# hyperconnect/TC-ResNet

Measured on AMD Instinct MI355X. Metric: utterances/sec (1 s@16 kHz) TCResNet8-1.0 forward, higher is better.
Workload: dtype f32; 1 GPU; TCResNet8-1.0 eval forward, waveform->softmax, batch 4096/GPU, 49x40 MFCC (40/20 ms, FFT 1024), 12 classes; global_batch=4096, parallelism=dp1 (utterance shards, no collective)

## Files before the change

### tc-resnet_amd/csrc/frontend_pk3.hip

```cpp
#include "frontend_plan.h"
#include "frontend_args.h"

namespace tcr {


namespace {

template <class T> __device__ __forceinline__ T lds_read_unpaired(const T* p) {
    const T v = *p;
    asm volatile("" ::: "memory");
    return v;
}

__device__ __forceinline__ void pk3_dft4(v2& a, v2& b, v2& c, v2& d) {
    const v2 t0 = a + c, t1 = a - c, t2 = b + d, t3 = b - d;
    a = t0 + t2;
    c = t0 - t2;
    b = c_submi(t1, t3);
    d = c_addmi(t1, t3);
}

__device__ __forceinline__ void pk3_dft16_tail(v2 (&v)[16]) {
    constexpr float C1 = 0.92387953251128673848f;
    constexpr float S1 = 0.38268343236508978178f;
    constexpr float R2 = 0.70710678118654752440f;
    v[1 + 4] = c_mulk(v[1 + 4], (v2){C1, -S1});
    v[1 + 8] = c_mulk(v[1 + 8], (v2){R2, -R2});
    v[1 + 12] = c_mulk(v[1 + 12], (v2){S1, -C1});
    v[2 + 4] = c_mulk(v[2 + 4], (v2){R2, -R2});
    v[2 + 8] = c_submi((v2){0.f, 0.f}, v[2 + 8]);
    v[2 + 12] = c_mulk(v[2 + 12], (v2){-R2, -R2});
    v[3 + 4] = c_mulk(v[3 + 4], (v2){S1, -C1});
    v[3 + 8] = c_mulk(v[3 + 8], (v2){-R2, -R2});
    v[3 + 12] = c_mulk(v[3 + 12], (v2){-C1, S1});
#pragma unroll
    for (int k1 = 0; k1 < 4; ++k1) pk3_dft4(v[4 * k1], v[4 * k1 + 1], v[4 * k1 + 2], v[4 * k1 + 3]);
#pragma unroll
    for (int i = 0; i < 4; ++i)
#pragma unroll
        for (int j = i + 1; j < 4; ++j) {
            const v2 t = v[4 * i + j];
            v[4 * i + j] = v[4 * j + i];
            v[4 * j + i] = t;
        }
}

__device__ __forceinline__ void pk3_dft16(v2 (&v)[16]) {
#pragma unroll
    for (int n0 = 0; n0 < 4; ++n0) pk3_dft4(v[n0], v[n0 + 4], v[n0 + 8], v[n0 + 12]);
    pk3_dft16_tail(v);
}

template <int QV>
__device__ __forceinline__ void pk3_window_dft4(const v2 (&x)[QV], const v2 (&w)[QV], v2 (&v)[16]) {
#pragma clang fp contract(on)
    static_assert(QV >= 8 && QV <= 16, "inputs n0 and n0 + 4 of every 4-point DFT are live");
#pragma unroll
    for (int n0 = 0; n0 < 4; ++n0) {
        v2 t0, t1, t2, t3;
        if (n0 + 8 < QV) {
            const v2 c = x[n0 + 8] * w[n0 + 8];
            t0 = x[n0] * w[n0] + c;
            t1 = x[n0] * w[n0] - c;
        } else {
            t0 = t1 = x[n0] * w[n0];
        }
        if (n0 + 12 < QV) {
            const v2 d = x[n0 + 12] * w[n0 + 12];
            t2 = x[n0 + 4] * w[n0 + 4] + d;
            t3 = x[n0 + 4] * w[n0 + 4] - d;
        } else {
            t2 = t3 = x[n0 + 4] * w[n0 + 4];
        }
        v[n0] = t0 + t2;
        v[n0 + 8] = t0 - t2;
        v[n0 + 4] = c_submi(t1, t3);
        v[n0 + 12] = c_addmi(t1, t3);
    }
}

__device__ __forceinline__ void pk3_real_pair_power(v2 zk, v2 zn, v2 wmi, float& p_lo, float& p_hi) {
    const v2 A = c_addc(zk, zn), D = c_subc(zk, zn);
    const v2 C = c_mul(D, wmi);
    pk_sq_pair(A, C, p_lo, p_hi);
}

constexpr int kPk3Carry = 1;
constexpr int kPk3BandsReg = 2;
constexpr int kPk3ItemsReg = 4;
constexpr int pk3_round_policy(int nc, int qv) {
#ifdef TCR_PK3_POLICY
    return TCR_PK3_POLICY;
#endif
    if (nc == 512) return qv == 10 ? kPk3BandsReg | kPk3ItemsReg : 0;
    return qv == 16 ? kPk3ItemsReg : kPk3Carry | kPk3ItemsReg;
}

}

template <int NC, int QV, bool MAG, bool STREAM>
__global__ __launch_bounds__(256, 3) void frontend_pk3_kernel(const FrontendArgs a) {
    constexpr int LPF = NC / 16;
    constexpr int FPR = 256 / LPF;
    constexpr int FPWV = FPR / 4;
    constexpr int SUB = NC / 256;
    constexpr int NBINS = NC + 1;
    constexpr int NMEL = 64, NSEG = NMEL + 1;
    constexpr int RS = 9;
    constexpr int UNITSZ = 16 * RS;
    constexpr int TILEW = 4 * UNITSZ;
    constexpr int PLD = NBINS + (LPF >= 32 ? 31 : 15);
    static_assert(FPWV * PLD <= 2 * TILEW, "the power spectrum of a wave's frames lives in its tile space");
    constexpr int kMelItemBins = mel_item_bins(NC);
    constexpr int kPolicy = pk3_round_policy(NC, QV);
    constexpr bool kCarry = kPolicy & kPk3Carry, kBandsReg = kPolicy & kPk3BandsReg, kItemsReg = kPolicy & kPk3ItemsReg;
    constexpr int NIT = mel_items_fast(NC);
    constexpr int USZ = NIT + 8; static_assert(NIT + 3 <= USZ, "the log phase reads up to three cells from a band's first item");
    static_assert(mel_dummy_item(NC, NIT) < USZ, "the empty slots' cell lies inside the item-sum row");
    constexpr int TRIPS = mel_trips(NC);

    __shared__ v2 s_t[4 * TILEW];
    __shared__ v2 s_ud[4 * FPWV * USZ];
    __shared__ float s_lm[4 * NMEL * 16];
    __shared__ v4 s_wit[kMelItemBins / 2 * NIT];
    __shared__ int s_items[NIT];
    __shared__ int s_band[NMEL];
    __shared__ v2 s_wnd[QV * LPF];

    const int tid = threadIdx.x;
    const int wave = __builtin_amdgcn_readfirstlane(tid >> 6);
    {
        const float fold = MAG ? 0.5f : 0.25f;
        const v2* wit = reinterpret_cast<const v2*>(a.mel_wit);
        for (int i = tid; i < kMelItemBins / 2 * NIT; i += 256) {
            const int bp = i / NIT, it = i % NIT;
            const v2 w0 = wit[2 * bp * NIT + it] * fold, w1 = wit[(2 * bp + 1) * NIT + it] * fold;
            s_wit[i] = (v4){w0.x, w0.y, w1.x, w1.y};
        }
        for (int i = tid; i < NIT; i += 256) s_items[i] = a.mel_items[i];
        if (tid < NMEL) s_band[tid] = a.mel_ifirst[tid] | (a.mel_ifirst[tid + 1] << 8) | (a.mel_ifirst[tid + 2] << 16);
        for (int i = tid; i < QV * LPF; i += 256) {
            const int q = i / LPF, lfi = i % LPF;
            s_wnd[i] = *reinterpret_cast<const v2*>(a.window_sgn + 2 * (SUB * ((lfi & 15) + 16 * q) + (lfi >> 4)));
        }
    }
    const v2* tw256 = reinterpret_cast<const v2*>(a.tw256);
    const v2* tw_real = reinterpret_cast<const v2*>(a.tw_real);
    const v2* tw_combine = reinterpret_cast<const v2*>(a.tw_combine);
    v2 tw[16], twr[8], twc[8];
    float sgn;
    {
        const int lf = tid % LPF, l = tid & 15, h = l >> 3;
        sgn = h && (SUB == 1 || lf >= 16) ? -1.f : 1.f;
#pragma unroll
        for (int j = 0; j < 16; ++j) tw[j] = tw256[l * 16 + (j ^ (8 * h))];
#pragma unroll
        for (int i = 0; i < 8; ++i) {
            const int k = lf + LPF * i;
            const v2 w = tw_real[k];
            twr[i] = (v2){w.y, -w.x};
            twc[i] = (SUB == 2) ? tw_combine[k] * sgn : (v2){1.f, 0.f};
        }
    }
    const v2 wm = tw_real[NC / 2];
    const v2 twmid = (v2){wm.y, -wm.x};

    const float inv_frames = 1.0f / (float)a.n_frames;
    const int rounds = a.rounds;
    const int fpwv = rounds * FPWV;
    const int fpw = 4 * fpwv;
    v2 xa[QV];
    int ft = 0;
    const float* fsrc = a.wav;
    const int step_r = FPWV % a.n_frames;
    const ptrdiff_t step_src = (ptrdiff_t)(FPWV / a.n_frames) * a.n_samples + (ptrdiff_t)step_r * a.hop;
    const ptrdiff_t step_src_wrap = step_src + a.n_samples - (ptrdiff_t)a.n_frames * a.hop;
    auto frame_at = [&](int chunk, int rr) {
        const int tid = (int)threadIdx.x;
        const int lf = tid % LPF, u = lf >> 4, l = tid & 15, fw = (tid & 63) / LPF;
        int g = chunk * fpw + wave * fpwv + rr * FPWV + fw;
        g = min(g, a.total_frames - 1);
        int n = (int)(((float)g + 0.5f) * inv_frames);
        n += (n + 1) * a.n_frames <= g ? 1 : (n * a.n_frames > g ? -1 : 0);
        ft = g - n * a.n_frames;
        fsrc = a.wav + (size_t)n * a.n_samples + (size_t)ft * a.hop + 2 * (SUB * l + u);
    };
    auto frame_next = [&]() {
        const unsigned t = (unsigned)(ft + step_r), tm = t - (unsigned)a.n_frames;
        fsrc += tm < t ? step_src_wrap : step_src;
        ft = (int)min(t, tm);
    };
    auto load_frame = [&](v2 (&dst)[QV]) {
#pragma unroll
        for (int q = 0; q < QV; ++q) dst[q] = *reinterpret_cast<const v2*>(fsrc + 2 * SUB * 16 * q);
    };
    const int nchunks = (a.total_frames + fpw - 1) / fpw;
    frame_at(blockIdx.x, 0);
    load_frame(xa);
    __syncthreads();
    if (a.stagger > 0) {
        const int steps = (((int)blockIdx.x / a.stagger_div) * 4 + wave) * a.stagger;
        for (int i = 0; i < steps; ++i) __builtin_amdgcn_s_sleep(1);
    }

#pragma unroll 1
    for (int chunk = blockIdx.x; chunk < nchunks; chunk += gridDim.x) {
    const int tid = (int)threadIdx.x + opaque_zero();
    const int lane = tid & 63;
    const int lf = tid % LPF, u = lf >> 4, l = tid & 15, h = l >> 3;
    const int fw = lane / LPF;
    v2* T = s_t + wave * TILEW + (lane >> 4) * UNITSZ;
    float* Pw = reinterpret_cast<float*>(s_t + wave * TILEW);
    float* LM = s_lm + wave * (NMEL * 16);
    int item_d[kItemsReg ? TRIPS : 1], band_i[kBandsReg ? NMEL / LPF : 1];
    if (kItemsReg) {
#pragma unroll
        for (int tr = 0; tr < TRIPS; ++tr) item_d[kItemsReg ? tr : 0] = s_items[lf + LPF * tr];
    }
    if (kBandsReg) {
#pragma unroll
        for (int i = 0; i < NMEL / LPF; ++i) band_i[kBandsReg ? i : 0] = s_band[lf + LPF * i];
    }
#pragma unroll 1
    for (int r = 0; r < rounds; ++r) {
        v2 v[16];
        {
            const v2* wsrc = s_wnd + lf;
            v2 wnd[QV];
#pragma unroll
            for (int q = 0; q < QV; ++q) wnd[q] = lds_read_unpaired(wsrc + q * LPF);
            pk3_window_dft4<QV>(xa, wnd, v);
        }
        pk3_dft16_tail(v);
#pragma unroll
        for (int j = 0; j < 16; ++j) v[j] = c_mul(v[j], tw[j]);
        {
            v2* wa = T + (8 * h) * RS + (l & 7);
            v2* wb = T + (8 * (1 - h)) * RS + (l & 7);
            const v2* rd = T + l * RS;
#pragma unroll
            for (int j = 0; j < 8; ++j) wa[j * RS] = v[j];
            wave_sync();
#pragma unroll
            for (int c = 0; c < 8; ++c) v[c] = lds_read_unpaired(rd + c);
            wave_sync();
#pragma unroll
            for (int j = 0; j < 8; ++j) wb[j * RS] = v[8 + j];
            wave_sync();
#pragma unroll
            for (int c = 0; c < 8; ++c) v[8 + c] = lds_read_unpaired(rd + c);
        }
        pk3_dft16(v);
        const v2 s2 = (v2){sgn, sgn};
        if (SUB == 1) {
#pragma unroll
            for (int k1 = 1; k1 < 16; k1 += 2) v[k1] = v[k1] * s2;
        }
        wave_sync();
        {
            float* P = Pw + fw * PLD;
            const int partner = (lane & ~(LPF - 1)) | (SUB == 2 ? (l ? (16 * (1 - u) + 16 - l) : 16 * u) : ((16 - l) & 15));
            if (SUB == 2) {
#pragma unroll
                for (int i = 0; i < 8; ++i) {
                    float ex = v[2 * i].x, ey = v[2 * i].y, ox = v[2 * i + 1].x, oy = v[2 * i + 1].y;
                    row_swap(ex, ox, lane);
                    row_swap(ey, oy, lane);
                    const v2 t = c_mul((v2){ox, oy}, twc[i]);
                    const v2 e = (v2){ex, ey};
                    v[2 * i] = __builtin_elementwise_fma(e, s2, t);
                    v[2 * i + 1] = __builtin_elementwise_fma(e, s2, -t);
                }
            }
            float* Plo = P + lf;
            float* Phi = P + (NC - LPF * 7 - lf);
            v2 prev = v[0];
#pragma unroll
            for (int i2 = 0; i2 < 8; i2 += 2) {
                float plo[2], phi[2];
#pragma unroll
                for (int j = 0; j < 2; ++j) {
                    const int i = i2 + j;
                    const v2 zk = SUB == 2 ? v[2 * i] : v[i];
                    const v2 src = SUB == 2 ? v[15 - 2 * i] : v[15 - i];
                    const v2 g = (v2){lane_gather(src.x, partner), lane_gather(src.y, partner)};
                    const v2 zn = lf == 0 ? prev : g;
                    prev = g;
                    pk3_real_pair_power(zk, zn, twr[i], plo[j], phi[j]);
                    if (MAG) { plo[j] = sqrtf(plo[j]); phi[j] = sqrtf(phi[j]); }
                }
                Plo[LPF * i2] = plo[0];
                Plo[LPF * (i2 + 1)] = plo[1];
                Phi[LPF * (7 - i2)] = phi[0];
                Phi[LPF * (6 - i2)] = phi[1];
            }
            if (lf == 0) {
                const v2 z = SUB == 2 ? v[1] : v[8];
                float plo, phi;
                pk3_real_pair_power(z, z, twmid, plo, phi);
                if (MAG) plo = sqrtf(plo);
                P[NC / 2] = plo;
            }
            if (lf < PLD - NBINS) P[NBINS + lf] = 0.f;
        }
        {
            const bool jump = r + 1 == rounds;
            const int ch = jump ? chunk + (int)gridDim.x : chunk;
            if (ch < nchunks) {
                if (kCarry && !jump && (ch + 1) * fpw <= a.total_frames) frame_next();
                else frame_at(ch, jump ? 0 : r + 1);
                load_frame(xa);
            }
        }
        wave_sync();
        v2* UD = s_ud + (wave * FPWV + fw) * USZ;
        int bi_pre[NMEL / LPF];
#pragma unroll
        for (int i = 0; i < NMEL / LPF; ++i) bi_pre[i] = kBandsReg ? band_i[kBandsReg ? i : 0] : s_band[lf + LPF * i];
        {
            const float* P = Pw + fw * PLD;
#pragma unroll
            for (int tr = 0; tr < TRIPS; ++tr) {
                const int it = lf + LPF * tr;
                const int d = kItemsReg ? item_d[kItemsReg ? tr : 0] : s_items[it];
                const float* pk = P + (d & 1023);
                const v4* wk = s_wit + it;
                float p[kMelItemBins];
                v2 wv[kMelItemBins];
#pragma unroll
                for (int b = 0; b < kMelItemBins; ++b) p[b] = pk[b];
#pragma unroll
                for (int bp = 0; bp < kMelItemBins / 2; ++bp) {
                    const v4 w = wk[bp * NIT];
                    wv[2 * bp] = (v2){w.x, w.y};
                    wv[2 * bp + 1] = (v2){w.z, w.w};
                }
                v2 ud = (v2){0.f, 0.f};
#pragma unroll
                for (int b = 0; b < kMelItemBins; ++b) ud = __builtin_elementwise_fma(wv[b], (v2){p[b], p[b]}, ud);
                UD[(d >> 21) & 255] = ud;
            }
        }
        wave_sync();
        {
            const int c = r * FPWV + fw;
            constexpr int NB = NMEL / LPF;
            constexpr int MAXC = NC == 512 ? 3 : 2;
            float up[NB][MAXC], dn[NB][MAXC];
#pragma unroll
            for (int i = 0; i < NB; ++i) {
                const int bi = bi_pre[i];
                const int i0 = bi & 255, i1 = (bi >> 8) & 255;
#pragma unroll
                for (int cc = 0; cc < MAXC; ++cc) {
                    up[i][cc] = lds_read_unpaired(UD + i0 + cc).x;
                    dn[i][cc] = lds_read_unpaired(UD + i1 + cc).y;
                }
            }
#pragma unroll
            for (int i = 0; i < NB; ++i) {
                const int m = lf + LPF * i;
                const int bi = bi_pre[i];
                const int i0 = bi & 255, i1 = (bi >> 8) & 255, i2 = bi >> 16;
                float mel = 0.f;
#pragma unroll
                for (int cc = 0; cc < MAXC; ++cc) mel += i0 + cc < i1 ? up[i][cc] : 0.f;
                if (NC != 512) for (int it = i0 + MAXC; it < i1; ++it) mel += UD[it].x;
#pragma unroll
                for (int cc = 0; cc < MAXC; ++cc) mel += i1 + cc < i2 ? dn[i][cc] : 0.f;
                if (NC != 512) for (int it = i1 + MAXC; it < i2; ++it) mel += UD[it].y;
                LM[m * 16 + (c ^ ((m >> 1) & 15))] = fast_log(a.log_floor ? fmaxf(mel, 1e-12f) : mel + 1e-6f);
            }
        }
    }
    wave_sync();

    {
        const int kq = lane >> 4, col = lane & 15;
        const int g = chunk * fpw + wave * fpwv + col;
        const bool valid = col < fpwv && g < a.total_frames;
        const int gg = valid ? g : a.total_frames - 1;
        const int n = gg / a.n_frames;
        const int t = gg - n * a.n_frames;
        const int col0 = STREAM ? a.tp - 2 * kHalo - a.n_frames : 0;
        float* dst = a.out + (size_t)n * a.n_coef * a.tp + kHalo + col0 + t;
        if (a.no_dct) {
            for (int m = kq; m < a.n_coef; m += 4) {
                if (valid) {
                    float* row = dst + (size_t)m * a.tp;
                    row[0] = LM[m * 16 + (col ^ ((m >> 1) & 15))];
                    if (t == 0 && (!STREAM || col0 == 0)) { row[-4] = 0.f; row[-3] = 0.f; row[-2] = 0.f; row[-1] = 0.f; }
                    if (t == a.n_frames - 1) { row[1] = 0.f; row[2] = 0.f; row[3] = 0.f; row[4] = 0.f; }
                }
            }
        } else {
            constexpr int CT = NMEL / 16;
            const int ntile = (a.n_coef + 15) >> 4;
            const int c0 = col ^ (kq >> 1);
            float bv[NMEL / 4];
#pragma unroll
            for (int st = 0; st < NMEL / 4; ++st) bv[st] = LM[(4 * st + kq) * 16 + (c0 ^ ((2 * st) & 14))];
#pragma unroll
            for (int ct = 0; ct < CT; ++ct) {
                if (ct < ntile) {
                    float av[NMEL / 4];
#pragma unroll
                    for (int st = 0; st < NMEL / 4; ++st) av[st] = a.dct_tab[(ct * (NMEL / 4) + st) * 64 + lane];
                    v4 acc = (v4){0.f, 0.f, 0.f, 0.f};
#pragma unroll
                    for (int st = 0; st < NMEL / 4; ++st) acc = __builtin_amdgcn_mfma_f32_16x16x4f32(av[st], bv[st], acc, 0, 0, 0);
                    if (valid) {
#pragma unroll
                        for (int rr = 0; rr < 4; ++rr) {
                            const int c = 16 * ct + 4 * kq + rr;
                            if (c < a.n_coef) {
                                float* row = dst + (size_t)c * a.tp;
                                row[0] = acc[rr];
                                if (t == 0 && (!STREAM || col0 == 0)) { row[-4] = 0.f; row[-3] = 0.f; row[-2] = 0.f; row[-1] = 0.f; }
                                if (t == a.n_frames - 1) { row[1] = 0.f; row[2] = 0.f; row[3] = 0.f; row[4] = 0.f; }
                            }
                        }
                    }
                }
            }
        }
    }
    }
}

int frontend_pk3_supports(int nc, int win, int n_items) {
    const int sub = nc / 256;
    if ((nc != 256 && nc != 512) || (win & 1) || (win / 2) % (16 * sub) != 0) return 0;
    if (n_items < 0 || n_items > mel_items_fast(nc)) return 0;
    const int qv = win / (32 * sub);
    return (qv == 10 || qv == 15 || qv == 16) ? 1 : 0;
}

template <bool STREAM>
static int launch_pk3(int nc, const FrontendArgs& a0, int n_items, hipStream_t s) {
    const int sub = nc / 256;
    if (!a0.aligned || (a0.win & 1) || (a0.win / 2) % (16 * sub) != 0) return 1;
    if (a0.total_frames >= (1 << 23)) return 1;
    if (n_items < 0 || n_items > mel_items_fast(nc)) return 1;
    const int qv = a0.win / (32 * sub);
    FrontendArgs a = a0;
    int grid = 0;
    {
        const int fpr = 4096 / nc, max_rounds = 64 / fpr, slots = 3 * device_cus();
        int best = max_rounds;
        float best_cost = 3.4e38f;
        const int r_min = ceil_div(a.total_frames, fpr) <= slots / 2 ? 1 : (max_rounds + 1) / 2;
        for (int r = max_rounds; r >= r_min; --r) {
            const int chunks = ceil_div(a.total_frames, r * fpr);
            const int full = chunks / slots, rest = chunks % slots;
            const float gens = (float)full + (rest == 0 ? 0.f : (3 * rest <= slots ? 0.45f : (3 * rest <= 2 * slots ? 0.75f : 1.f)));
            const float cost = gens * ((float)r + 1.45f);
            if (cost < best_cost * 0.995f) { best_cost = cost; best = r; }
        }
        const int knob = tune_get(TCR_TUNE_FRONTEND);
        if (knob >= 10 && knob < 30) best = min(max(knob - 10, 1), max_rounds);
        if (a0.rounds > 0) best = min(a0.rounds, max_rounds);
        a.rounds = best;
        grid = min(ceil_div(a.total_frames, best * fpr), slots);
        const int cap = tune_get(TCR_TUNE_FE_GRID);
        if (cap > 0) grid = min(grid, cap);
        a.stagger = tune_get(TCR_TUNE_FE_STAGGER);
        a.stagger_div = device_cus();
    }
#define TCR_FPK3(NC_, QV_)                                                                                          \
    if (nc == NC_ && qv == QV_) {                                                                                   \
        if (a.magnitude) hipLaunchKernelGGL((frontend_pk3_kernel<NC_, QV_, true, STREAM>), dim3(grid), dim3(256), 0, s, a); \
        else hipLaunchKernelGGL((frontend_pk3_kernel<NC_, QV_, false, STREAM>), dim3(grid), dim3(256), 0, s, a);            \
        return check_launch("frontend_pk3_kernel");                                                                 \
    }
    TCR_FPK3(512, 10)
    TCR_FPK3(256, 15)
    TCR_FPK3(512, 16)
    TCR_FPK3(256, 16)
    TCR_FPK3(256, 10)
    TCR_FPK3(512, 15)
#undef TCR_FPK3
    return 1;
}

int launch_frontend_pk3(int nc, const FrontendArgs& a, int n_items, hipStream_t s) { return launch_pk3<false>(nc, a, n_items, s); }
int launch_frontend_pk3_stream(int nc, const FrontendArgs& a, int n_items, hipStream_t s) { return launch_pk3<true>(nc, a, n_items, s); }

}

#include "stream.hip"
#include "scan.hip"
#include "sweep.hip"
#include "detect_grid.hip"
#include "scan_select.hip"
#include "mine.hip"
#include "compose.hip"
#include "phrase.hip"
#include "capture.hip"
#include "resample.hip"
#include "stream_cascade.hip"
```

Measured before the change: 19.69 million utterances/s.

## Prefetch DCT table before wave sync and specialize MFMA DCT tiles per coefficient count

The DCT epilogue now issues global loads of the DCT table ahead of the wave barrier and keeps a sliding prefetch window, so load latency overlaps the sync and the MFMA chain. The number of coefficient tiles becomes a template constant, and for QV==10 several tiles are computed together. Halo zeroing moves out of the per-row store loop into a single wave-uniform guarded block, and the frame index division uses a precomputed reciprocal. The rounds cost model also gets a smaller fixed overhead term, which shifts the chosen rounds and grid size. Optional cycle-counter stamps are added behind a compile flag. The cost is higher register pressure from the prefetched table values.

New measurement: 19.82 million utterances/s (median of 6 runs). Within noise of the previous version (+0.7%).

```diff
diff --git a/tc-resnet_amd/csrc/frontend_pk3.hip b/tc-resnet_amd/csrc/frontend_pk3.hip
--- a/tc-resnet_amd/csrc/frontend_pk3.hip
+++ b/tc-resnet_amd/csrc/frontend_pk3.hip
@@ -95,6 +95,24 @@
     if (nc == 512) return qv == 10 ? kPk3BandsReg | kPk3ItemsReg : 0;
     return qv == 16 ? kPk3ItemsReg : kPk3Carry | kPk3ItemsReg;
 }
+
+template <int N> struct pk3_int { static constexpr int value = N; };
+
+#ifdef TCR_PK3_STAMP
+__device__ long long* g_pk3_stamps = nullptr;
+#define TCR_PK3_STAMP_AT(var) const long long var = (long long)__builtin_readcyclecounter()
+#define TCR_PK3_STAMP_OUT(chunk, wave, lane, t0, t1)                                                \
+    do {                                                                                            \
+        const long long t2_ = (long long)__builtin_readcyclecounter();                              \
+        if ((lane) == 0 && g_pk3_stamps) {                                                          \
+            long long* sp_ = g_pk3_stamps + ((size_t)(chunk) * 4 + (wave)) * 4;                     \
+            sp_[0] = (t0); sp_[1] = (t1); sp_[2] = t2_; sp_[3] = (long long)blockIdx.x;             \
+        }                                                                                           \
+    } while (0)
+#else
+#define TCR_PK3_STAMP_AT(var) ((void)0)
+#define TCR_PK3_STAMP_OUT(chunk, wave, lane, t0, t1) ((void)0)
+#endif
 
 }
 
@@ -221,6 +239,7 @@
 #pragma unroll
         for (int i = 0; i < NMEL / LPF; ++i) band_i[kBandsReg ? i : 0] = s_band[lf + LPF * i];
     }
+    TCR_PK3_STAMP_AT(ts_chunk);
 #pragma unroll 1
     for (int r = 0; r < rounds; ++r) {
         v2 v[16];
@@ -373,57 +392,100 @@
             }
         }
     }
-    wave_sync();
+    TCR_PK3_STAMP_AT(ts_dct);
 
     {
         const int kq = lane >> 4, col = lane & 15;
-        const int g = chunk * fpw + wave * fpwv + col;
+        const int g0 = chunk * fpw + wave * fpwv;
+        const int g = g0 + col;
         const bool valid = col < fpwv && g < a.total_frames;
         const int gg = valid ? g : a.total_frames - 1;
-        const int n = gg / a.n_frames;
+        const int n = fast_div(gg, a.n_frames, inv_frames);
         const int t = gg - n * a.n_frames;
         const int col0 = STREAM ? a.tp - 2 * kHalo - a.n_frames : 0;
+        const bool lead = !STREAM || col0 == 0;
         float* dst = a.out + (size_t)n * a.n_coef * a.tp + kHalo + col0 + t;
+        const int cols = min(fpwv, a.total_frames - g0);
+        const int t0 = __builtin_amdgcn_readfirstlane(t);
+        const bool halo = cols > 0 && ((lead && t0 == 0) || t0 + cols >= a.n_frames);
         if (a.no_dct) {
+            wave_sync();
+            const float z = (float)opaque_zero();
             for (int m = kq; m < a.n_coef; m += 4) {
                 if (valid) {
                     float* row = dst + (size_t)m * a.tp;
                     row[0] = LM[m * 16 + (col ^ ((m >> 1) & 15))];
-                    if (t == 0 && (!STREAM || col0 == 0)) { row[-4] = 0.f; row[-3] = 0.f; row[-2] = 0.f; row[-1] = 0.f; }
-                    if (t == a.n_frames - 1) { row[1] = 0.f; row[2] = 0.f; row[3] = 0.f; row[4] = 0.f; }
+                    if (t == 0 && lead) { row[-4] = z; row[-3] = z; row[-2] = z; row[-1] = z; }
+                    if (t == a.n_frames - 1) { row[1] = z; row[2] = z; row[3] = z; row[4] = z; }
                 }
             }
         } else {
-            constexpr int CT = NMEL / 16;
-            const int ntile = (a.n_coef + 15) >> 4;
-            const int c0 = col ^ (kq >> 1);
-            float bv[NMEL / 4];
-#pragma unroll
-            for (int st = 0; st < NMEL / 4; ++st) bv[st] = LM[(4 * st + kq) * 16 + (c0 ^ ((2 * st) & 14))];
-#pragma unroll
-            for (int ct = 0; ct < CT; ++ct) {
-                if (ct < ntile) {
-                    float av[NMEL / 4];
-#pragma unroll
-                    for (int st = 0; st < NMEL / 4; ++st) av[st] = a.dct_tab[(ct * (NMEL / 4) + st) * 64 + lane];
-                    v4 acc = (v4){0.f, 0.f, 0.f, 0.f};
-#pragma unroll
-                    for (int st = 0; st < NMEL / 4; ++st) acc = __builtin_amdgcn_mfma_f32_16x16x4f32(av[st], bv[st], acc, 0, 0, 0);
+            auto tiles = [&](auto nt) {
+                constexpr int NT = decltype(nt)::value, NST = NMEL / 4;
+                constexpr int CP = QV == 10 ? NT : 1;
+                constexpr int AHEAD = CP > 1 ? 24 / CP : (NC == 512 && QV != 10 ? 8 : NST);
+                const float* at = a.dct_tab + lane;
+                float av[CP][NST];
+                auto request = [&](int cg, int st) {
+#pragma unroll
+                    for (int ct = 0; ct < CP; ++ct) av[ct][st] = at[((cg + ct) * NST + st) * 64];
+                };
+#pragma unroll
+                for (int st = 0; st < AHEAD; ++st) request(0, st);
+                wave_sync();
+                const int c0 = col ^ (kq >> 1);
+                float bv[NST];
+#pragma unroll
+                for (int st = 0; st < NST; ++st) bv[st] = LM[(4 * st + kq) * 16 + (c0 ^ ((2 * st) & 14))];
+                const size_t pitch = (size_t)a.tp;
+                float* base = dst + (size_t)(4 * kq) * pitch;
+                const int nrow = a.n_coef - 4 * kq;
+#pragma unroll
+                for (int cg = 0; cg < NT; cg += CP) {
+                    if (cg > 0) {
+#pragma unroll
+                        for (int st = 0; st < AHEAD; ++st) request(cg, st);
+                    }
+                    v4 acc[CP];
+#pragma unroll
+                    for (int ct = 0; ct < CP; ++ct) acc[ct] = (v4){0.f, 0.f, 0.f, 0.f};
+#pragma unroll
+                    for (int st = 0; st < NST; ++st) {
+                        if (st + AHEAD < NST) request(cg, st + AHEAD);
+#pragma unroll
+                        for (int ct = 0; ct < CP; ++ct) acc[ct] = __builtin_amdgcn_mfma_f32_16x16x4f32(av[ct][st], bv[st], acc[ct], 0, 0, 0);
+                    }
                     if (valid) {
 #pragma unroll
-                        for (int rr = 0; rr < 4; ++rr) {
-                            const int c = 16 * ct + 4 * kq + rr;
-                            if (c < a.n_coef) {
-                                float* row = dst + (size_t)c * a.tp;
-                                row[0] = acc[rr];
-                                if (t == 0 && (!STREAM || col0 == 0)) { row[-4] = 0.f; row[-3] = 0.f; row[-2] = 0.f; row[-1] = 0.f; }
-                                if (t == a.n_frames - 1) { row[1] = 0.f; row[2] = 0.f; row[3] = 0.f; row[4] = 0.f; }
-                            }
-                        }
+                        for (int ct = 0; ct < CP; ++ct)
+#pragma unroll
+                            for (int rr = 0; rr < 4; ++rr)
+                                if (cg + ct < NT - 1 || 16 * (cg + ct) + rr < nrow) base[(size_t)(16 * (cg + ct) + rr) * pitch] = acc[ct][rr];
                     }
                 }
-            }
-        }
+                if (halo) {
+                    const bool zlo = valid && lead && t == 0, zhi = valid && t == a.n_frames - 1;
+                    if (zlo || zhi) {
+                        const float z = (float)opaque_zero();
+                        for (int r16 = 0; r16 < 16 * NT; r16 += 16)
+#pragma unroll
+                            for (int rr = 0; rr < 4; ++rr)
+                                if (r16 + rr < nrow) {
+                                    float* row = base + (size_t)(r16 + rr) * pitch;
+                                    if (zlo) { row[-4] = z; row[-3] = z; row[-2] = z; row[-1] = z; }
+                                    if (zhi) { row[1] = z; row[2] = z; row[3] = z; row[4] = z; }
+                                }
+                    }
+                }
+            };
+            switch ((a.n_coef + 15) >> 4) {
+                case 1: tiles(pk3_int<1>{}); break;
+                case 2: tiles(pk3_int<2>{}); break;
+                case 3: tiles(pk3_int<3>{}); break;
+                default: tiles(pk3_int<4>{}); break;
+            }
+        }
+        TCR_PK3_STAMP_OUT(chunk, wave, lane, ts_chunk, ts_dct);
     }
     }
 }
@@ -454,7 +516,7 @@
             const int chunks = ceil_div(a.total_frames, r * fpr);
             const int full = chunks / slots, rest = chunks % slots;
             const float gens = (float)full + (rest == 0 ? 0.f : (3 * rest <= slots ? 0.45f : (3 * rest <= 2 * slots ? 0.75f : 1.f)));
-            const float cost = gens * ((float)r + 1.45f);
+            const float cost = gens * ((float)r + 0.9f);
             if (cost < best_cost * 0.995f) { best_cost = cost; best = r; }
         }
         const int knob = tune_get(TCR_TUNE_FRONTEND);
@@ -485,6 +547,13 @@
 
 int launch_frontend_pk3(int nc, const FrontendArgs& a, int n_items, hipStream_t s) { return launch_pk3<false>(nc, a, n_items, s); }
 int launch_frontend_pk3_stream(int nc, const FrontendArgs& a, int n_items, hipStream_t s) { return launch_pk3<true>(nc, a, n_items, s); }
+
+#ifdef TCR_PK3_STAMP
+extern "C" int tcr_pk3_stamp_buffer(void* dev_buf) {
+    long long* p = static_cast<long long*>(dev_buf);
+    return (int)hipMemcpyToSymbol(HIP_SYMBOL(g_pk3_stamps), &p, sizeof(p));
+}
+#endif
 
 }
 
```
